# Jiang-Muyun/PointNet12

Measured on AMD Instinct MI355X. Metric: points/sec fwd+bwd, PointNet2 SemSeg B=16x4096 pts, higher is better.
Workload: dtype f32 (wide-layer products: exact bf16x3 operand splits, 6 bf16 MFMAs per fp32 product, fp32 accumulate)

## Files before the change

### pointnet12_amd/csrc/mlp_res.hip

```cpp
#include "mlp_loaders.h"
#include "split_bf16.h"
#include <algorithm>

int pn2_wide_fwd(const float *X, int ldx, const float *in_affine, const float *W, int ldw, const float *bias, float *Y, int ldy,
                 int64_t P, int K, int N, double *stats, LazyBn lz, hipStream_t s, int64_t *rows_done, int Kpool,
                 const float *pool_gamma, float *pool_ws);

namespace {

constexpr int RES_BM = 64;

struct ResPlan {
    signed char dx_rb[8], dx_cj[8];
    signed char dw_cj[8], dw_q0[8], dw_q1[8];
};

inline bool make_res_plan(int CI_T, ResPlan *out) {
    ResPlan p;
    int load[8], next_q[4] = {0, 0, 0, 0};
    for (int w = 0; w < 8; ++w) { p.dx_rb[w] = p.dx_cj[w] = -1; p.dw_cj[w] = 0; p.dw_q0[w] = p.dw_q1[w] = 0; load[w] = 0; }
    if (CI_T < 1 || CI_T > 4) return false;
    for (int i = 0; i < 2 * CI_T; ++i) { p.dx_rb[i] = (signed char)(i & 1); p.dx_cj[i] = (signed char)(i >> 1); load[i] = 2; }
    const int target = CI_T > 2 ? CI_T : 2;
    for (int pass = 0; pass < 2; ++pass)
// ... 686 lines not shown
                        const float4 a0 = xr[0], a1 = xr[1], a2 = xr[2];
                        g0[0] = __builtin_fmaf(dz, a0.x, g0[0]); g0[FUSE0 ? 1 : 0] = __builtin_fmaf(dz, a0.y, g0[FUSE0 ? 1 : 0]);
                        g0[FUSE0 ? 2 : 0] = __builtin_fmaf(dz, a0.z, g0[FUSE0 ? 2 : 0]); g0[FUSE0 ? 3 : 0] = __builtin_fmaf(dz, a0.w, g0[FUSE0 ? 3 : 0]);
                        g0[FUSE0 ? 4 : 0] = __builtin_fmaf(dz, a1.x, g0[FUSE0 ? 4 : 0]); g0[FUSE0 ? 5 : 0] = __builtin_fmaf(dz, a1.y, g0[FUSE0 ? 5 : 0]);
                        g0[FUSE0 ? 6 : 0] = __builtin_fmaf(dz, a1.z, g0[FUSE0 ? 6 : 0]); g0[FUSE0 ? 7 : 0] = __builtin_fmaf(dz, a1.w, g0[FUSE0 ? 7 : 0]);
                        g0[FUSE0 ? 8 : 0] = __builtin_fmaf(dz, a2.x, g0[FUSE0 ? 8 : 0]); g0[FUSE0 ? 9 : 0] = __builtin_fmaf(dz, a2.y, g0[FUSE0 ? 9 : 0]);
                        g0[FUSE0 ? 10 : 0] = __builtin_fmaf(dz, a2.z, g0[FUSE0 ? 10 : 0]); g0[FUSE0 ? 11 : 0] = __builtin_fmaf(dz, a2.w, g0[FUSE0 ? 11 : 0]);
                    } else {
#if defined(PN2_EXP_NOSTORE)
                        if (dz == 1.2345e-33f) xb[offx] = dz;
#elif defined(PN2_EXP_PLAINSTORE)
                        xb[offx] = dz;
#else
                        PN2_STREAM_STORE(dz, xb + offx);
#endif
                    }
                    offx += ((r & 3) == 3 ? 5u : 1u) * (unsigned)ldxo;
                }
                if (MASKED) { st0 += (double)s0; st1 += (double)s1; }
                RSTAMP(4)
            }
            chunk += G;
            buf ^= 1;
        };
        while (chunk < chunks) {
            iter(D2 ? raw1 : raw0);
            if (chunk >= chunks) break;
            iter(raw0);
        }
        RSTAMP_FLUSH(wave)
        RABS(wave, 2)
        if (!DXW) {
#pragma unroll
            for (int j = 0; j < TW; ++j) {
                const int e = (wave - CI_T) + j * NDW;
                if (e < NTILE) {
                    const int mb = e / CI_T, nb = e - mb * CI_T;
#pragma unroll
                    for (int r = 0; r < 16; ++r)
                        atomicAdd(dW + (int64_t)(mb * 32 + acc_row(r, lh)) * lddw + nb * 32 + l31, accw[DXW ? 0 : j][r]);
                }
            }
        } else if (MASKED && red_p != nullptr) {
            st0 += __shfl_xor(st0, 32, 64);
            st1 += __shfl_xor(st1, 32, 64);
            if (lh == 0) {
                double *rep = red_p + (size_t)(blockIdx.x % PN2_STAT_REPLICAS) * 2 * Ci;
                atomicAdd(rep + ecol, st0);
                atomicAdd(rep + Ci + ecol, st1);
            }
        }
        if (DXW && FUSE0) {
#pragma unroll
            for (int j = 0; j < (DXW && FUSE0 ? 12 : 1); ++j) g0[j] += __shfl_xor(g0[j], 32, 64);
            if (lh == 0) {
                float *pr = part0 + ((size_t)(blockIdx.x % PN2_CF_REPL) * Ci + ecol) * 16;
#pragma unroll
                for (int j = 0; j < (DXW && FUSE0 ? 12 : 1); ++j) atomicAdd(pr + j, g0[j]);
            }
        }
    };
    if (has_dx) run(pn2_true{}); else run(pn2_false{});
    RABS(wave, 3)
}

template <int CO_T, int CI_T, bool POOLED, bool MASKED, bool FUSE0 = false>
int launch_split_bwd_res(ResDy dy, const float *Yp, int ldp, const float *aff_p, const float *W, int ldw, int64_t tiles, float *dX, int ldxo,
                         double *red_p, float *dW, int lddw, hipStream_t s, const float *X0 = nullptr, int ld0 = 0, float *part0 = nullptr) {
    constexpr int Co = 32 * CO_T, Ci = 32 * CI_T;
    constexpr size_t lds = 2 * 6 * (size_t)(32 * 256) + sizeof(float) * (2 * 32 * (Ci + 4) + 8 * Co + 6 * Ci + (FUSE0 ? 2 * 32 * 12 : 0)) +
                           (CO_T == 4 && CI_T < 4 ? (size_t)CI_T * (Co / 16) * 1024 : 0);
    static_assert(lds <= 160 * 1024, "LDS");
    if ((reinterpret_cast<uintptr_t>(dy.Y) & 15) != 0 || (reinterpret_cast<uintptr_t>(Yp) & 15) != 0) return PN2_EUNSUPPORTED;
    auto kern = split_bwd_res_kernel<CO_T, CI_T, POOLED, MASKED, FUSE0>;
    static Pn2PerDevice raised;
    if (pn2_raise_dynamic_lds(reinterpret_cast<const void *>(kern), raised) != PN2_OK) return PN2_ELAUNCH;
    const int64_t chunks = tiles * (RES_BM / 32), cap = pn2_num_cus();
    PN2_NOTE_KERNEL(kern);
    hipLaunchKernelGGL(kern, dim3((unsigned)(chunks < cap ? chunks : cap)), dim3(512), lds, s, dy, Yp, ldp, aff_p, W, ldw, chunks, dX, ldxo,
                       red_p, dW, lddw, X0, ld0, part0);
    return pn2_launch_status();
}

template <int CO_T, int CI_T>
__global__ __launch_bounds__(512, 1) void split_bwd_cf_kernel(const float *dZp, const int32_t *arg, int ldo, int kshift, const float *W2 ,
                                                              const float *Yp, int ldp, const float *aff_p, int64_t chunks, float *dX, int ldxo, double *red_p,
                                                              float *slab) {
    constexpr int Co = 32 * CO_T, Ci = 32 * CI_T, BP = 32, QD = Co / 4, QP = Ci / 4, LDP = Ci + 4;
    constexpr int PANEL = BP * 256, BUF = 6 * PANEL;
    constexpr int KBX = Co / 16, KBM = Ci / 16, KBT = KBX + KBM;
    constexpr int NS = 8 - CI_T - 1, NTS = 64 * NS;
    constexpr int NGT = CI_T * (CI_T + 1) / 2, LDT = Co + Ci + 4;
    static_assert(NS >= CO_T, "one staging wave per D column");
    constexpr int RPP = NTS / QD, IT_D = (BP + RPP - 1) / RPP, IT_P = (BP * QP + NTS - 1) / NTS;
    static_assert(NTS % QD == 0, "one channel quad of D per staging thread");
    unsigned char *lds_b = reinterpret_cast<unsigned char *>(res_lds);
    float *Yps = res_lds + (2 * BUF) / 4;
    float *xtab = Yps + 2 * BP * LDP;
    const int t = threadIdx.x, lane = t & 63, wave = __builtin_amdgcn_readfirstlane(t >> 6), l31 = lane & 31, lh = lane >> 5;
    const int G = gridDim.x;
    RABS(wave, 0)
    for (int i = t; i < 3 * Ci; i += 512) { const float v = aff_p[i]; xtab[i] = v; xtab[3 * Ci + i] = i < Ci ? v : -v; }

    const bool has_dx = wave < CI_T, is_gram = wave == CI_T;
    const int ecol = (has_dx ? wave : 0) * 32 + l31;
    const int ts = wave <= CI_T ? 0 : t - 64 * (CI_T + 1);
    struct Raw { float4 z; int4 a; float4 p[IT_P]; };
    Raw raw;
    auto p_item = [&](int i, int &row, int &q) { const int idx = (NTS * (i + 1) > BP * QP) ? min(ts + NTS * i, BP * QP - 1) : ts + NTS * i; row = idx / QP; q = idx - row * QP; };
    auto fetch = [&](int64_t chunk) {
        const unsigned m0 = (unsigned)(chunk < chunks ? chunk : chunks - 1) * BP;
        const unsigned o = (m0 >> kshift) * (unsigned)ldo + 4u * (unsigned)(ts % QD);
        raw.z = ld4(dZp + o);
        raw.a = ld4i(arg + o);
#pragma unroll
        for (int i = 0; i < IT_P; ++i) {
            int row, q;
            p_item(i, row, q);
            raw.p[i] = ld4(Yp + ((m0 + (unsigned)row) * (unsigned)ldp + 4u * (unsigned)q));
        }
    };
    auto store_split = [&](unsigned char *img, int row, int q, const float4 v) {
        unsigned h0, m0, l0, h1, m1, l1;
        split2(v.x, v.y, h0, m0, l0);
        split2(v.z, v.w, h1, m1, l1);
        const unsigned o = tr_img_off(row, q >> 1) + 8u * (unsigned)(q & 1);
        *reinterpret_cast<uint2 *>(img + o) = make_uint2(h0, h1);
        *reinterpret_cast<uint2 *>(img + o + PANEL) = make_uint2(m0, m1);
        *reinterpret_cast<uint2 *>(img + o + 2 * PANEL) = make_uint2(l0, l1);
    };
    auto stage = [&](int64_t chunk, int buf) {
        unsigned char *ia = lds_b + buf * BUF, *ib = ia + 3 * PANEL;
        float *yp = Yps + buf * (BP * LDP);
        const unsigned m0 = (unsigned)(chunk < chunks ? chunk : chunks - 1) * BP;
        const int kbase = (int)(m0 & ((1u << kshift) - 1u));
        const int par = (int)(chunk & 1);
        const float *xt = xtab + par * (3 * Ci);
        const float lim = par ? -INFINITY : INFINITY;
        {
            unsigned h0, m0_, l0, h1, m1, l1;
            split2(raw.z.x, raw.z.y, h0, m0_, l0);
            split2(raw.z.z, raw.z.w, h1, m1, l1);
            const unsigned sm2 = par ? 0x80008000u : 0u;
            h0 ^= sm2; m0_ ^= sm2; l0 ^= sm2; h1 ^= sm2; m1 ^= sm2; l1 ^= sm2;
            const int q = ts % QD, r0 = ts / QD;
            const int4 a = raw.a;
#pragma unroll
            for (int i = 0; i < IT_D; ++i) {
                const int row = (RPP * (i + 1) > BP) ? min(r0 + RPP * i, BP - 1) : r0 + RPP * i;
                const int k = kbase + row;
                const unsigned k0 = (a.x == k ? 0x0000ffffu : 0u) | (a.y == k ? 0xffff0000u : 0u);
                const unsigned k1 = (a.z == k ? 0x0000ffffu : 0u) | (a.w == k ? 0xffff0000u : 0u);
                const unsigned o = tr_img_off(row, q >> 1) + 8u * (unsigned)(q & 1);
                *reinterpret_cast<uint2 *>(ia + o) = make_uint2(h0 & k0, h1 & k1);
                *reinterpret_cast<uint2 *>(ia + o + PANEL) = make_uint2(m0_ & k0, m1 & k1);
                *reinterpret_cast<uint2 *>(ia + o + 2 * PANEL) = make_uint2(l0 & k0, l1 & k1);
            }
        }
#pragma unroll
        for (int i = 0; i < IT_P; ++i) {
            int row, q;
            p_item(i, row, q);
            float4 x = raw.p[i];
            *reinterpret_cast<float4 *>(&yp[row * LDP + 4 * q]) = x;
            const float4 mu = *reinterpret_cast<const float4 *>(&xt[4 * q]), sc = *reinterpret_cast<const float4 *>(&xt[Ci + 4 * q]);
            const float4 be = *reinterpret_cast<const float4 *>(&xt[2 * Ci + 4 * q]);
            x.x = __builtin_amdgcn_fmed3f(bn_act(x.x, mu.x, sc.x, be.x), 0.f, lim); x.y = __builtin_amdgcn_fmed3f(bn_act(x.y, mu.y, sc.y, be.y), 0.f, lim);
            x.z = __builtin_amdgcn_fmed3f(bn_act(x.z, mu.z, sc.z, be.z), 0.f, lim); x.w = __builtin_amdgcn_fmed3f(bn_act(x.w, mu.w, sc.w, be.w), 0.f, lim);
            store_split(ib, row, q, x);
        }
    };
    auto raw_landed = [&]() {
        asm volatile("" : "+v"(raw.z.x), "+v"(raw.z.y), "+v"(raw.z.z), "+v"(raw.z.w));
        asm volatile("" : "+v"(raw.a.x), "+v"(raw.a.y), "+v"(raw.a.z), "+v"(raw.a.w));
#pragma unroll
        for (int i = 0; i < IT_P; ++i) asm volatile("" : "+v"(raw.p[i].x), "+v"(raw.p[i].y), "+v"(raw.p[i].z), "+v"(raw.p[i].w));
    };
    const int g16 = lane >> 4, j16 = lane & 15, tq = j16 >> 2, tp = j16 & 3;
    auto frag_t = [&](const unsigned char *img, int cblk, int pb) {
        const int c0 = (cblk * 32 + 16 * (g16 & 1)) >> 3;
        SplitFrag f;
#pragma unroll
        for (int r2 = 0; r2 < 2; ++r2) {
            const int row = 16 * pb + 8 * (g16 >> 1) + 4 * r2 + tq;
            const unsigned o = tr_img_off(row, c0 + (tp >> 1)) + 8u * (unsigned)(tp & 1);
            const pn2_s16x4 v = __builtin_amdgcn_ds_read_tr16_b64_v4i16(
                reinterpret_cast<__attribute__((address_space(3))) pn2_s16x4 *>((__attribute__((address_space(3))) unsigned char *)(img) + o));
            const uint2 u = __builtin_bit_cast(uint2, v);
            f.u[2 * r2] = u.x; f.u[2 * r2 + 1] = u.y;
        }
        return f;
    };

    if (has_dx) {
        SplitFrag wh[KBT], wm[KBT], wl[KBM];
        uint4 *wl_lds = reinterpret_cast<uint4 *>(xtab + 6 * Ci) + (size_t)wave * KBX * 64 + lane;
        {
            float v[KBT][8];
#pragma unroll
            for (int kb = 0; kb < KBT; ++kb)
#pragma unroll
                for (int e = 0; e < 8; ++e) v[kb][e] = W2[(16 * kb + 8 * lh + e) * Ci + ecol];
#pragma unroll
            for (int kb = 0; kb < KBT; ++kb) {
                SplitFrag lo;
#pragma unroll
                for (int e = 0; e < 4; ++e) split2(v[kb][2 * e], v[kb][2 * e + 1], wh[kb].u[e], wm[kb].u[e], lo.u[e]);
                if (kb < KBX) wl_lds[kb * 64] = lo.q; else wl[kb < KBX ? 0 : kb - KBX] = lo;
            }
        }
        Affine a(aff_p, Ci);
        const float emu = a.mean[ecol], esc = a.scale[ecol], ebe = a.beta[ecol], eis = a.invstd[ecol];
        const float eh = W2[(Co + Ci) * Ci + ecol];
        double st0 = 0.0, st1 = 0.0, st2 = 0.0;
        int64_t chunk = blockIdx.x;
        int buf = 0;
        __syncthreads();
        RABS(wave, 1)
        RSTAMP_DECL
        while (chunk < chunks) {
            __syncthreads();
            RSTAMP(2)
            const unsigned char *ia = lds_b + buf * BUF, *ib = ia + 3 * PANEL;
            f32x16 acc, acc2;
#pragma unroll
            for (int r = 0; r < 16; ++r) { acc[r] = 0.f; acc2[r] = 0.f; }
#ifndef PN2_X_CF_NODXM
#pragma unroll
            for (int kb = 0; kb < KBT; ++kb) {
                const unsigned char *img = kb < KBX ? ia : ib;
                const unsigned o = tr_img_off(l31, 2 * (kb < KBX ? kb : kb - KBX) + lh);
                SplitFrag ah, am, al, wlo;
                ah.q = *reinterpret_cast<const uint4 *>(img + o);
                am.q = *reinterpret_cast<const uint4 *>(img + o + PANEL);
                al.q = *reinterpret_cast<const uint4 *>(img + o + 2 * PANEL);
                if (kb < KBX) wlo.q = wl_lds[kb * 64]; else wlo = wl[kb < KBX ? 0 : kb - KBX];
                acc = __builtin_amdgcn_mfma_f32_32x32x16_bf16(al.v, wh[kb].v, acc, 0, 0, 0);
                acc2 = __builtin_amdgcn_mfma_f32_32x32x16_bf16(ah.v, wlo.v, acc2, 0, 0, 0);
                acc = __builtin_amdgcn_mfma_f32_32x32x16_bf16(am.v, wm[kb].v, acc, 0, 0, 0);
                acc2 = __builtin_amdgcn_mfma_f32_32x32x16_bf16(am.v, wh[kb].v, acc2, 0, 0, 0);
                acc = __builtin_amdgcn_mfma_f32_32x32x16_bf16(ah.v, wm[kb].v, acc, 0, 0, 0);
                acc2 = __builtin_amdgcn_mfma_f32_32x32x16_bf16(ah.v, wh[kb].v, acc2, 0, 0, 0);
            }
#endif
#ifdef PN2_STAMP
            { float a0_ = acc[0] + acc2[0]; asm volatile("" : "+v"(a0_)); }
#endif
            RSTAMP(3)
#ifdef PN2_X_CF_NOEPI
            if (acc[0] == 1.2345e-33f) dX[0] = acc2[1];
            chunk += G; buf ^= 1;
            continue;
#endif
            const float *yq = Yps + buf * (BP * LDP) + (4 * lh) * LDP + ecol;
            float yv[16];
#pragma unroll
            for (int r = 0; r < 16; ++r) yv[r] = yq[((r & 3) + 8 * (r >> 2)) * LDP];
            float *xb = dX + ((size_t)chunk * BP + 4 * lh) * (unsigned)ldxo;
            unsigned offx = (unsigned)ecol;
            asm volatile("" : "+v"(offx));
            float s0 = 0.f, s1 = 0.f, s2 = 0.f;
            const unsigned sgn = (unsigned)(chunk & 1) << 31;
#pragma unroll
            for (int r = 0; r < 16; ++r) {
                const float y = yv[r];
                const float x = bn_act(y, emu, esc, ebe);
                float dz = __uint_as_float(__float_as_uint(acc[r] + acc2[r]) ^ sgn) + eh;
                dz = x > 0.f ? dz : 0.f;
                s0 += dz;
                s1 = __builtin_fmaf(dz, (y - emu) * eis, s1);
                s2 += fmaxf(x, 0.f);
                PN2_STREAM_STORE(dz, xb + offx);
                offx += ((r & 3) == 3 ? 5u : 1u) * (unsigned)ldxo;
            }
            st0 += (double)s0; st1 += (double)s1; st2 += (double)s2;
            RSTAMP(4)
            chunk += G;
            buf ^= 1;
        }
        RSTAMP_FLUSH(wave)
        RABS(wave, 2)
        st0 += __shfl_xor(st0, 32, 64);
        st1 += __shfl_xor(st1, 32, 64);
        st2 += __shfl_xor(st2, 32, 64);
        if (lh == 0) {
            if (red_p != nullptr) {
                double *rep = red_p + (size_t)(blockIdx.x % PN2_STAT_REPLICAS) * 2 * Ci;
                atomicAdd(rep + ecol, st0);
                atomicAdd(rep + Ci + ecol, st1);
            }
            slab[(size_t)blockIdx.x * (Ci * LDT) + (size_t)ecol * LDT + Co + Ci] = (float)st2;
        }
    } else {
        constexpr int PA[6] = {2, 0, 1, 1, 0, 0}, PB[6] = {0, 2, 1, 0, 1, 0};
        auto mm2 = [&](f32x16 &c0, const SplitFrag (&a0)[3], const SplitFrag (&b0)[3], f32x16 &c1, const SplitFrag (&a1)[3], const SplitFrag (&b1)[3]) {
#pragma unroll
            for (int q = 0; q < 6; ++q) {
                c0 = __builtin_amdgcn_mfma_f32_32x32x16_bf16(a0[PA[q]].v, b0[PB[q]].v, c0, 0, 0, 0);
                c1 = __builtin_amdgcn_mfma_f32_32x32x16_bf16(a1[PA[q]].v, b1[PB[q]].v, c1, 0, 0, 0);
            }
        };
        auto mm1 = [&](f32x16 &c0, const SplitFrag (&a0)[3], const SplitFrag (&b0)[3]) {
#pragma unroll
            for (int q = 0; q < 6; ++q) c0 = __builtin_amdgcn_mfma_f32_32x32x16_bf16(a0[PA[q]].v, b0[PB[q]].v, c0, 0, 0, 0);
        };
        auto frag3 = [&](const unsigned char *img, int blk, int pb, SplitFrag (&f)[3]) {
            f[0] = frag_t(img, blk, pb); f[1] = frag_t(img + PANEL, blk, pb); f[2] = frag_t(img + 2 * PANEL, blk, pb);
        };
        float *sl = slab + (size_t)blockIdx.x * (Ci * LDT);
        if (is_gram) {
            f32x16 accg[NGT];
#pragma unroll
            for (int j = 0; j < NGT; ++j)
#pragma unroll
                for (int r = 0; r < 16; ++r) accg[j][r] = 0.f;
            int64_t chunk = blockIdx.x;
            int buf = 0;
            __syncthreads();
            RABS(wave, 1)
            RSTAMP_DECL
            while (chunk < chunks) {
                __syncthreads();
                RSTAMP(2)
#ifndef PN2_X_CF_NOT
                const unsigned char *ib = lds_b + buf * BUF + 3 * PANEL;
#pragma unroll
                for (int pb = 0; pb < BP / 16; ++pb) {
                    SplitFrag fx[CI_T][3];
#pragma unroll
                    for (int i = 0; i < CI_T; ++i) frag3(ib, i, pb, fx[i]);
                    if constexpr (CI_T == 1) {
                        mm1(accg[0], fx[0], fx[0]);
                    } else if constexpr (CI_T == 2) {
                        mm2(accg[0], fx[0], fx[0], accg[1], fx[0], fx[1]);
                        mm1(accg[2], fx[1], fx[1]);
                    } else {
                        static_assert(CI_T <= 3, "Gram tiles");
                        mm2(accg[0], fx[0], fx[0], accg[1], fx[0], fx[1]);
                        mm2(accg[2], fx[1], fx[1], accg[3], fx[0], fx[2]);
                        mm2(accg[4], fx[1], fx[2], accg[5], fx[2], fx[2]);
                    }
                }
#endif
                RSTAMP(3)
                chunk += G;
                buf ^= 1;
            }
            RSTAMP_FLUSH(wave)
            RABS(wave, 2)
#pragma unroll
            for (int j = 0; j < CI_T; ++j)
#pragma unroll
                for (int i = 0; i <= j; ++i) {
                    const f32x16 &acc = accg[j * (j + 1) / 2 + i];
#pragma unroll
                    for (int r = 0; r < 16; ++r) sl[(i * 32 + acc_row(r, lh)) * LDT + Co + j * 32 + l31] = acc[r];
                    if (i != j) {
#pragma unroll
                        for (int r = 0; r < 16; ++r) sl[(j * 32 + l31) * LDT + Co + i * 32 + acc_row(r, lh)] = acc[r];
                    }
                }
        } else {
            f32x16 accw[CI_T];
#pragma unroll
            for (int j = 0; j < CI_T; ++j)
#pragma unroll
                for (int r = 0; r < 16; ++r) accw[j][r] = 0.f;
            const int nb = wave - CI_T - 1 < CO_T ? wave - CI_T - 1 : -1;
            int64_t chunk = blockIdx.x;
            fetch(chunk);
            __syncthreads();
            stage(chunk, 0);
            fetch(chunk + G);
            raw_landed();
            int buf = 0;
            RABS(wave, 1)
            RSTAMP_DECL
            while (chunk < chunks) {
                __syncthreads();
                RSTAMP(2)
#ifndef PN2_X_CF_NOSTAGE
                stage(chunk + G, buf ^ 1);
#endif
                RSTAMP(0)
#ifndef PN2_X_CF_NOFETCH
                fetch(chunk + 2 * (int64_t)G);
#endif
                __builtin_amdgcn_sched_barrier(0);
                RSTAMP(1)
#ifndef PN2_X_CF_NOT
                if (nb >= 0) {
                    const unsigned char *ia = lds_b + buf * BUF, *ib = ia + 3 * PANEL;
#pragma unroll
                    for (int pb = 0; pb < BP / 16; ++pb) {
                        SplitFrag fb[3], fa0[3], fa1[3];
                        frag3(ia, nb, pb, fb);
                        frag3(ib, 0, pb, fa0);
                        if constexpr (CI_T >= 2) {
                            frag3(ib, 1, pb, fa1);
                            mm2(accw[0], fa0, fb, accw[CI_T >= 2 ? 1 : 0], fa1, fb);
                            if constexpr (CI_T == 3) {
                                frag3(ib, 2, pb, fa0);
                                mm1(accw[CI_T == 3 ? 2 : 0], fa0, fb);
                            }
                        } else {
                            mm1(accw[0], fa0, fb);
                        }
                    }
                }
#endif
                RSTAMP(3)
                chunk += G;
                buf ^= 1;
            }
            RSTAMP_FLUSH(wave)
            RABS(wave, 2)
            if (nb >= 0) {
#pragma unroll
                for (int i = 0; i < CI_T; ++i)
#pragma unroll
                    for (int r = 0; r < 16; ++r) sl[(i * 32 + acc_row(r, lh)) * LDT + nb * 32 + l31] = accw[i][r];
            }
        }
    }
    RABS(wave, 3)
}

__global__ __launch_bounds__(128) void cf_prep_kernel(LazyCoef lc, const float *coef, int ldc, const float *__restrict__ W, int ldw,
                                                      const float *__restrict__ bias, int Co, int Ci, float *__restrict__ W2) {
    __shared__ double fac[256];
    lazy_coef_prologue(lc);
    const float *c0 = coef, *q1 = coef + ldc, *q0 = coef + 2 * ldc, *mean = coef + 3 * ldc;
    const int r = blockIdx.x;
    if (r < Co) {
        for (int i = threadIdx.x; i < Ci; i += 128) W2[r * Ci + i] = c0[r] * W[(int64_t)r * ldw + i];
        return;
    }
    const int j = r - Co;
    for (int c = threadIdx.x; c < Co; c += 128)
        fac[c] = j == Ci ? ((double)q1[c] * ((double)bias[c] - (double)mean[c]) + (double)q0[c]) : (double)W[(int64_t)c * ldw + j] * (double)q1[c];
    __syncthreads();
    for (int i = threadIdx.x; i < Ci; i += 128) {
        double s0 = 0.0, s1 = 0.0, s2 = 0.0, s3 = 0.0;
#pragma unroll 4
        for (int c = 0; c < Co; c += 4) {
            s0 += fac[c] * (double)W[(int64_t)c * ldw + i];
            s1 += fac[c + 1] * (double)W[(int64_t)(c + 1) * ldw + i];
            s2 += fac[c + 2] * (double)W[(int64_t)(c + 2) * ldw + i];
            s3 += fac[c + 3] * (double)W[(int64_t)(c + 3) * ldw + i];
        }
        W2[r * Ci + i] = (float)((s0 + s1) + (s2 + s3));
    }
}

__global__ __launch_bounds__(256) void cf_finish_kernel(const float *__restrict__ slab, int nslab, int Co, int Ci, const float *coef, int ldc,
                                                        const float *__restrict__ W, int ldw, const float *__restrict__ bias,
                                                        float *__restrict__ dW, int lddw) {
    extern __shared__ double cf_row[];
    const int i = blockIdx.x, LDT = Co + Ci + 4, NQ = LDT / 4;
    const int q = threadIdx.x & 63, sg = threadIdx.x >> 6;
    double a0 = 0.0, a1 = 0.0, a2 = 0.0, a3 = 0.0;
    if (q < NQ) {
        const float *p = slab + (size_t)i * LDT + 4 * q;
        const size_t ss = (size_t)Ci * LDT;
        int w = sg;
        for (; w + 28 < nslab; w += 32) {
            float4 v[8];
#pragma unroll
            for (int e = 0; e < 8; ++e) v[e] = ld4(p + (size_t)(w + 4 * e) * ss);
#pragma unroll
            for (int e = 0; e < 8; ++e) { a0 += (double)v[e].x; a1 += (double)v[e].y; a2 += (double)v[e].z; a3 += (double)v[e].w; }
        }
        for (; w < nslab; w += 4) {
            const float4 v = ld4(p + (size_t)w * ss);
            a0 += (double)v.x; a1 += (double)v.y; a2 += (double)v.z; a3 += (double)v.w;
        }
        double *d = cf_row + sg * LDT + 4 * q;
        d[0] = a0; d[1] = a1; d[2] = a2; d[3] = a3;
    }
    __syncthreads();
    for (int n = threadIdx.x; n < LDT; n += 256) cf_row[n] = (cf_row[n] + cf_row[LDT + n]) + (cf_row[2 * LDT + n] + cf_row[3 * LDT + n]);
    __syncthreads();
    const float *c0 = coef, *q1 = coef + ldc, *q0 = coef + 2 * ldc, *mean = coef + 3 * ldc;
    const double sx = cf_row[Co + Ci];
    for (int c = threadIdx.x; c < Co; c += 256) {
        double dot = 0.0;
        for (int j = 0; j < Ci; ++j) dot += (double)W[(int64_t)c * ldw + j] * cf_row[Co + j];
        const double g = (double)c0[c] * cf_row[c] + (double)q1[c] * (dot + ((double)bias[c] - (double)mean[c]) * sx) + (double)q0[c] * sx;
        dW[(int64_t)c * lddw + i] += (float)g;
    }
}

template <int CO_T, int CI_T>
int launch_split_bwd_cf(const float *dZp, const int32_t *arg, int ldo, int kshift, const float *coef, LazyCoef lc, const float *W, int ldw,
                        const float *bias, const float *Yp, int ldp, const float *aff_p, int64_t P, float *dX, int ldxo, double *red_p,
                        float *dW, int lddw, float *scratch, hipStream_t s) {
    constexpr int Co = 32 * CO_T, Ci = 32 * CI_T, LDT = Co + Ci + 4;
    constexpr size_t lds = 2 * 6 * (size_t)(32 * 256) + sizeof(float) * (2 * 32 * (Ci + 4) + 6 * Ci) + (size_t)CI_T * (Co / 16) * 1024;
    static_assert(lds <= 160 * 1024, "LDS");
    auto kern = split_bwd_cf_kernel<CO_T, CI_T>;
    static Pn2PerDevice raised;
    if (pn2_raise_dynamic_lds(reinterpret_cast<const void *>(kern), raised) != PN2_OK) return PN2_ELAUNCH;
    float *W2 = scratch, *slab = scratch + (((Co + Ci + 1) * Ci + 63) & ~63);
    const int64_t chunks = P / 32, cap = pn2_num_cus() < 256 ? pn2_num_cus() : 256;
    const int grid = (int)(chunks < cap ? chunks : cap);
    hipLaunchKernelGGL(cf_prep_kernel, dim3(Co + Ci + 1), dim3(128), 0, s, lc, coef, (Co + 3) & ~3, W, ldw, bias, Co, Ci, W2);
    PN2_NOTE_KERNEL(kern);
    hipLaunchKernelGGL(kern, dim3((unsigned)grid), dim3(512), lds, s, dZp, arg, ldo, kshift, W2, Yp, ldp, aff_p, chunks, dX, ldxo, red_p, slab);
    hipLaunchKernelGGL(cf_finish_kernel, dim3(Ci), dim3(256), sizeof(double) * 4 * LDT, s, slab, grid, Co, Ci, coef, (Co + 3) & ~3, W, ldw, bias,
                       dW, lddw);
    return pn2_launch_status();
}

#define PN2_RES_CASE(CO, CI, POOL, MASKED)                                                                                \
    if (Co == CO && Ci == CI)                                                                                              \
        return launch_bwd_res<CO / 32, CI / 32, POOL, MASKED>(dy, Yp, ldp, aff_p, W, ldw, tiles, dX, ldxo, red_p, dW, lddw, s);

int dispatch_bwd_res(int Kpool, bool masked, int Co, int Ci, ResDy dy, const float *Yp, int ldp, const float *aff_p, const float *W,
                     int ldw, int64_t tiles, float *dX, int ldxo, double *red_p, float *dW, int lddw, hipStream_t s) {
    if (pn2_opt(PN2_OPT_SPLIT) && pn2_opt(PN2_OPT_SPLIT_RES)) {
#define PN2_SPLIT_RES_CASE(CO, CI, POOLED, MASKED)                                                                        \
        if (Co == CO && Ci == CI) {                                                                                        \
            const int rc = launch_split_bwd_res<CO / 32, CI / 32, POOLED, MASKED>(dy, Yp, ldp, aff_p, W, ldw, tiles, dX, ldxo, red_p, dW, lddw, s); \
            if (rc != PN2_EUNSUPPORTED) return rc;                                                                         \
        }
        const bool all = pn2_opt(PN2_OPT_SPLIT_RES) >= 2;
        if (Kpool == 0 && masked) {
            if (all) { PN2_SPLIT_RES_CASE(32, 32, false, true) }
            PN2_SPLIT_RES_CASE(64, 64, false, true) PN2_SPLIT_RES_CASE(96, 64, false, true)
            if (tiles >= pn2_opt(PN2_OPT_SPLIT_RES_MIN_TILES_128)) { PN2_SPLIT_RES_CASE(128, 128, false, true) }
        } else if (Kpool == 0) {
            if (tiles >= pn2_opt(PN2_OPT_SPLIT_RES_MIN_TILES_128)) { PN2_SPLIT_RES_CASE(128, 128, false, false) }
        } else if (masked && Kpool % 32 == 0) {
            if (all) { PN2_SPLIT_RES_CASE(64, 32, true, true) }
            PN2_SPLIT_RES_CASE(128, 64, true, true) PN2_SPLIT_RES_CASE(128, 96, true, true)
        }
#undef PN2_SPLIT_RES_CASE
    }
    if (Kpool == 0 && masked) {
        PN2_RES_CASE(32, 32, 0, true) PN2_RES_CASE(64, 64, 0, true) PN2_RES_CASE(96, 64, 0, true)
        if (tiles >= 4096) { PN2_RES_CASE(128, 128, 0, true) }
    } else if (Kpool == 0) {
        if (tiles >= 4096) { PN2_RES_CASE(128, 128, 0, false) }
    } else if (masked && Kpool % 64 == 0) {
        PN2_RES_CASE(128, 64, 1, true) PN2_RES_CASE(128, 96, 1, true)
    } else if (masked && Kpool == 32) {
        PN2_RES_CASE(64, 32, 2, true) PN2_RES_CASE(128, 64, 2, true)
    }
    return PN2_EUNSUPPORTED;
}

struct ResPool {
    float2 *rec;
    const float *gamma;
    int ldp, U;
    LazyBn lz;
};

template <int K_T, int N_T, bool ACT, int POOL>
__global__ __launch_bounds__(512, 2) void fwd_res_kernel(const float *__restrict__ X, int ldx, const float *aff ,
                                                         const float *__restrict__ W, int ldw, const float *__restrict__ bias,
                                                         float *__restrict__ Y, int ldy, int64_t slabs, double *__restrict__ stats,
                                                         ResPool pool) {
    constexpr int K = 32 * K_T, N = 32 * N_T, LDA = K + 4, QK = K / 4, IT = 32 * QK / 64;
    const int NW = blockDim.x >> 6;
    float *Ws = res_lds;
    float *atab = Ws + N * LDA;
    const int t = threadIdx.x, lane = t & 63, wave = __builtin_amdgcn_readfirstlane(t >> 6), l31 = lane & 31, lh = lane >> 5;
    float *Ab = atab + 3 * K + wave * (32 * LDA);
    RABS(wave, 0)

    lazy_bn_prologue(pool.lz);
    for (int i = t; i < N * QK; i += blockDim.x) {
        const int n = i / QK, q = i - n * QK;
        const float *src = W + (int64_t)n * ldw + 4 * q;
        float4 v;
        if ((ldw & 3) == 0 && (reinterpret_cast<uintptr_t>(W) & 15) == 0) v = ld4(src);
        else v = make_float4(src[0], src[1], src[2], src[3]);
        *reinterpret_cast<float4 *>(&Ws[n * LDA + 4 * q]) = v;
    }
    if (ACT)
        for (int i = t; i < 3 * K; i += blockDim.x) atab[i] = aff[i];
    float bj[N_T];
// ... 326 lines not shown

extern "C" int pn2_bn_pool_select(const float *pool_ws, const float *affine, int64_t G, int C, float *out, int ldo, int32_t *arg,
                                  const pn2_bn_lazy *lazy, pn2_stream_t stream) {
    PN2_CHECK_ARG(lazy_bn_ok(lazy, affine, C));
    PN2_CHECK_ARG(pool_ws && affine && out && arg && G > 0 && C > 0 && C % 32 == 0 && ldo >= C && ldo % 4 == 0 &&
                  (reinterpret_cast<uintptr_t>(pool_ws) & 15) == 0 && (reinterpret_cast<uintptr_t>(out) & 15) == 0);
    const int64_t n = G * (C >> 2);
    int64_t blocks = pn2_cdiv(n, 256);
    const int64_t cap = (int64_t)pn2_num_cus() * 8;
    if (blocks > cap) blocks = cap;
    hipLaunchKernelGGL(bn_pool_select_kernel, dim3((unsigned)blocks), dim3(256), 0, pn2_s(stream),
                       reinterpret_cast<const float2 *>(pool_ws), C, affine, C, G, C, out, ldo, arg, make_lazy_bn(lazy));
    return pn2_launch_status();
}

extern "C" int pn2_conv1x1_bwd(const float *dZ, int ldz, const float *dZp, int ldo, const int32_t *arg, int Kpool, const float *Y,
                               int ldy, const float *coef, const float *W, int ldw, const float *prev_Y, int ld_prev,
                               const float *prev_affine, float *dXout, int ldxo, double *prev_red, float *dW, int lddw,
                               int64_t P, int C_out, int C_in, const pn2_bn_coef_lazy *coef_lazy, pn2_stream_t stream) {
    PN2_CHECK_ARG(Y && coef && W && prev_Y && dXout && dW && P > 0 && P < (1LL << 31) && res_shape_ok(C_out, C_in));
    PN2_CHECK_ARG(lazy_coef_ok(coef_lazy, coef, C_out));
    PN2_CHECK_ARG(dZ != nullptr || (dZp && arg && Kpool > 0));
    PN2_CHECK_ARG(ldw >= C_in && lddw >= C_in && ldy % 4 == 0 && ldy >= C_out && ld_prev % 4 == 0 && ld_prev >= C_in && ldxo >= C_in);
    PN2_CHECK_ARG(prev_affine != nullptr || prev_red == nullptr);
    hipStream_t s = pn2_s(stream);
    const int kshift = dZ ? 0 : pow2_shift(Kpool);
    PN2_CHECK_ARG(dZ ? (ldz == ldy) : (kshift >= 0 && ldo % 4 == 0 && ldo >= C_out && prev_affine != nullptr && P % Kpool == 0));
    int64_t tiles = P / RES_BM, P_full = tiles * RES_BM;
    int rc = PN2_OK;
    const int64_t ld_max = std::max(std::max((int64_t)ldy, (int64_t)ld_prev), std::max((int64_t)ldxo, dZ ? (int64_t)ldz : (int64_t)ldo));
    if (P * ld_max >= (1LL << 32)) { tiles = 0; P_full = 0; }
    if (tiles > 0) {
        ResDy dy{dZ, dZp, arg, ldo, kshift, Y, ldy, coef, make_lazy_coef(coef_lazy)};
        rc = dispatch_bwd_res(dZ ? 0 : Kpool, prev_affine != nullptr, C_out, C_in, dy, prev_Y, ld_prev, prev_affine, W, ldw, tiles, dXout, ldxo,
                              prev_red, dW, lddw, s);
        if (rc == PN2_EUNSUPPORTED) { rc = PN2_OK; tiles = 0; P_full = 0; }
        else coef_lazy = nullptr;
    }
    if (rc != PN2_OK || P_full == P) return rc;
    const int64_t tail = P - P_full;
    const int64_t g_off = dZ ? 0 : (P_full / Kpool) * ldo;
    const float *dZt = dZ ? dZ + P_full * ldz : nullptr;
    const float *dZpt = dZ ? nullptr : dZp + g_off;
    const int32_t *argt = dZ ? nullptr : arg + g_off;
    rc = pn2_conv1x1_dgrad(dZt, ldz, dZpt, ldo, argt, Kpool, Y + P_full * ldy, ldy, coef, W, ldw, prev_affine ? prev_Y + P_full * ld_prev : nullptr,
                           ld_prev, prev_affine, dXout + P_full * ldxo, ldxo, prev_red, tail, C_out, C_in, nullptr, coef_lazy, stream);
    if (rc != PN2_OK) return rc;
    return pn2_conv1x1_wgrad(dZt, ldz, dZpt, ldo, argt, Kpool, Y + P_full * ldy, ldy, coef, prev_Y + P_full * ld_prev, ld_prev, prev_affine,
                             dW, lddw, nullptr, tail, C_out, C_in, nullptr, stream);
}

static bool cf_shape(int C_out, int C_in) { return C_out == 128 && (C_in == 96 || C_in == 64); }

extern "C" int pn2_conv1x1_bwd_cf_supported(int64_t P, int C_out, int C_in, int Kpool) {
    if (!(pn2_opt(PN2_OPT_SPLIT) && pn2_opt(PN2_OPT_SPLIT_RES) && pn2_opt(PN2_OPT_POOL_CF))) return 0;
    if (!pn2_res_supported(P, C_out, C_in) || !cf_shape(C_out, C_in)) return 0;
    if (C_in == 64 && pn2_opt(PN2_OPT_POOL_CF) < 2) return 0;
    if (Kpool < 32 || (Kpool & (Kpool - 1)) != 0 || P % Kpool != 0) return 0;
    if (P * (int64_t)std::max(C_out, C_in) >= (1LL << 32)) return 0;
    return 1;
}

extern "C" int64_t pn2_conv1x1_bwd_cf_scratch_bytes(int C_out, int C_in) {
    if (!cf_shape(C_out, C_in)) return 0;
    const int64_t w2 = (((int64_t)(C_out + C_in + 1) * C_in + 63) & ~63LL);
    return 4 * (w2 + 256LL * C_in * (C_out + C_in + 4));
}

extern "C" int pn2_conv1x1_bwd_cf(const float *dZp, int ldo, const int32_t *arg, int Kpool, const float *coef, const float *W, int ldw,
                                  const float *bias, const float *prev_Y, int ld_prev, const float *prev_affine, float *dXout, int ldxo,
                                  double *prev_red, float *dW, int lddw, int64_t P, int C_out, int C_in, const pn2_bn_coef_lazy *coef_lazy,
                                  float *scratch, pn2_stream_t stream) {
    PN2_CHECK_ARG(dZp && arg && coef && W && bias && prev_Y && prev_affine && dXout && dW && scratch && P > 0 && P < (1LL << 31));
    PN2_CHECK_ARG(lazy_coef_ok(coef_lazy, coef, C_out));
    PN2_CHECK_ARG(ldw >= C_in && lddw >= C_in && ld_prev % 4 == 0 && ld_prev >= C_in && ldxo >= C_in && ldo % 4 == 0 && ldo >= C_out);
    PN2_CHECK_ARG((reinterpret_cast<uintptr_t>(scratch) & 255) == 0 && (reinterpret_cast<uintptr_t>(prev_Y) & 15) == 0 &&
                  (reinterpret_cast<uintptr_t>(dZp) & 15) == 0 && (reinterpret_cast<uintptr_t>(arg) & 15) == 0);
    if (!pn2_conv1x1_bwd_cf_supported(P, C_out, C_in, Kpool)) return PN2_EUNSUPPORTED;
    const int64_t ld_max = std::max(std::max((int64_t)ld_prev, (int64_t)ldxo), (int64_t)ldo);
    if (P * ld_max >= (1LL << 32)) return PN2_EUNSUPPORTED;
    const int kshift = pow2_shift(Kpool);
    const LazyCoef lc = make_lazy_coef(coef_lazy);
    hipStream_t s = pn2_s(stream);
    if (C_in == 96) return launch_split_bwd_cf<4, 3>(dZp, arg, ldo, kshift, coef, lc, W, ldw, bias, prev_Y, ld_prev, prev_affine, P, dXout, ldxo, prev_red, dW, lddw, scratch, s);
    return launch_split_bwd_cf<4, 2>(dZp, arg, ldo, kshift, coef, lc, W, ldw, bias, prev_Y, ld_prev, prev_affine, P, dXout, ldxo, prev_red, dW, lddw, scratch, s);
}

extern "C" int pn2_conv1x1_bwd_first_supported(int64_t P, int C_out, int C_in, int N0) {
    if (!(pn2_opt(PN2_OPT_SPLIT) && pn2_opt(PN2_OPT_SPLIT_RES) && pn2_opt(PN2_OPT_FUSE_FIRST))) return 0;
    if (!pn2_res_supported(P, C_out, C_in) || P % 64 != 0 || N0 < 1 || N0 > 12) return 0;
    if (P * (int64_t)std::max(C_out, C_in) >= (1LL << 32)) return 0;
    return (C_out == 96 && C_in == 64) || (C_out == 64 && C_in == 64);
}

extern "C" int pn2_conv1x1_bwd_first(const float *dZ, int ldz, const float *Y, int ldy, const float *coef, const float *W, int ldw,
                                     const float *prev_Y, int ld_prev, const float *prev_affine, double *prev_red, float *dW, int lddw,
                                     const float *X0, int ld0, int N0, void *cf_scratch, int64_t P, int C_out, int C_in,
                                     const pn2_bn_coef_lazy *coef_lazy, pn2_stream_t stream) {
    PN2_CHECK_ARG(dZ && Y && coef && W && prev_Y && prev_affine && prev_red && dW && X0 && cf_scratch && P > 0 && P < (1LL << 31));
    PN2_CHECK_ARG(lazy_coef_ok(coef_lazy, coef, C_out));
    PN2_CHECK_ARG(ldz == ldy && ldw >= C_in && lddw >= C_in && ldy % 4 == 0 && ldy >= C_out && ld_prev % 4 == 0 && ld_prev >= C_in);
    PN2_CHECK_ARG(ld0 % 4 == 0 && ld0 >= 12 && (reinterpret_cast<uintptr_t>(X0) & 15) == 0 && (reinterpret_cast<uintptr_t>(cf_scratch) & 15) == 0);
    if (!pn2_conv1x1_bwd_first_supported(P, C_out, C_in, N0)) return PN2_EUNSUPPORTED;
    if (P * (int64_t)std::max((int64_t)ldy, std::max((int64_t)ld_prev, (int64_t)ld0)) >= (1LL << 32)) return PN2_EUNSUPPORTED;
    float *part0 = reinterpret_cast<float *>(reinterpret_cast<double *>(cf_scratch) + PN2_CF_REPL * 256);
    ResDy dy{dZ, nullptr, nullptr, 0, 0, Y, ldy, coef, make_lazy_coef(coef_lazy)};
    const int64_t tiles = P / RES_BM;
    hipStream_t s = pn2_s(stream);
    if (C_out == 96) return launch_split_bwd_res<3, 2, false, true, true>(dy, prev_Y, ld_prev, prev_affine, W, ldw, tiles, nullptr, 0, prev_red, dW, lddw, s, X0, ld0, part0);
    return launch_split_bwd_res<2, 2, false, true, true>(dy, prev_Y, ld_prev, prev_affine, W, ldw, tiles, nullptr, 0, prev_red, dW, lddw, s, X0, ld0, part0);
}
```

### pointnet12_amd/csrc/pn2_common.h

```cpp
#pragma once
#include <hip/hip_runtime.h>
#include <stdint.h>
#include <mutex>
#include <set>
#include <utility>
#include "../../include/pn2.h"

#define PN2_WAVE 64
#define PN2_CF_REPL 8

#ifdef PN2_PLAIN_STORES
#define PN2_STREAM_STORE(value, ptr) (*(ptr) = (value))
#else
#define PN2_STREAM_STORE(value, ptr) __builtin_nontemporal_store((value), (ptr))
#endif

#define PN2_CHECK_ARG(cond) \
    do {                    \
        if (!(cond)) return PN2_EINVAL; \
    } while (0)

static inline int pn2_launch_status() { return hipGetLastError() == hipSuccess ? PN2_OK : PN2_ELAUNCH; }

static inline hipStream_t pn2_s(pn2_stream_t s) { return reinterpret_cast<hipStream_t>(s); }

static inline int64_t pn2_cdiv(int64_t a, int64_t b) { return (a + b - 1) / b; }

#define PN2_OPTION_LIST(X) \
    X(FPS_ROWS_MIN_PPT, 24)  \
    X(FPS_ROWMAP, 2)  \
    X(FPS_SINGLE_MAX, 24576)  \
    X(FPS_PIECE, 0)  \
    X(FPS_COOP, 1)  \
    X(FPS_PRUNE, 1)  \
    X(BQ_ORDER, 1)  \
    X(FEWROW_MAX_TILES, 1024)  \
    X(FEWROW_MAX_TILES_DGRAD, 512)  \
    X(FEWROW_KS, 0)  \
    X(NT_CFG, 0)  \
    X(NT_SMALL_DEPTH, 1)  \
    X(NT_NSPLIT, 1)  \
    X(TN_SPLITDIV, 1)  \
    X(TN_CFG, 0)  \
    X(TN_NARROW, 1)  \
    X(TN_SMALLP, 65536)  \
    X(TN_SMALL_DEPTH, 2)  \
    X(CF_WGS_PER_CU, 2)  \
    X(WGRAD_SKINNY, 1)  \
    X(BWD_PAIR, 1)  \
    X(RES, 1)  \
    X(RES_MIN_ROWS, 32768)  \
    X(RES_HALF, 1)  \
    X(WIDE, 1)  \
    X(WIDE_MIN_ROWS, 65536)  \
    X(SPLIT, 1)  \
    X(SPLIT_WGRAD, 1)  \
    X(SPLIT_K256, 1)  \
    X(SPLIT_NARROW, 1)  \
    X(SPLIT_RES, 1)  \
    X(FUSE_FIRST, 1)  \
    X(SPLIT_WG2, 1)  \
    X(POOL_CF, 2)  \
    X(SPLIT_RES_MIN_TILES_128, 1024)  \
    X(SPLIT_MIN_ROWS_128, 98304)  \
    X(RING, 0)  \
    X(WIDE_POOL, 1)  \
    X(WIDE_ADB196, 1)  \
    X(WIDE_WGRAD, 1)  \
    X(WIDE_WGRAD_MIN_ROWS, 131072)  \
    X(WGRAD_TWO_PHASE, 0)  \
    X(WGRAD_TWO_PHASE_ALL, 0)  \
    X(SEG_CHUNK, 0)

enum Pn2Option {
#define PN2_X(name, dflt) PN2_OPT_##name,
    PN2_OPTION_LIST(PN2_X)
#undef PN2_X
    PN2_OPT_COUNT
};
extern int pn2_option_table[PN2_OPT_COUNT];
static inline int pn2_opt(int id) { return __atomic_load_n(&pn2_option_table[id], __ATOMIC_RELAXED); }

extern thread_local const void *pn2_last_kernel_fn;
#define PN2_NOTE_KERNEL(...) (pn2_last_kernel_fn = reinterpret_cast<const void *>(__VA_ARGS__))

#define PN2_MAX_DEVICES 16
static inline int pn2_device_slot() {
    int dev = 0;
    if (hipGetDevice(&dev) != hipSuccess || dev < 0) dev = 0;
    return dev < PN2_MAX_DEVICES ? dev : PN2_MAX_DEVICES - 1;
}

static inline int pn2_num_cus() {
    static int cus[PN2_MAX_DEVICES] = {0};
    const int slot = pn2_device_slot();
    if (cus[slot] == 0) {
        int dev = 0;
        hipDeviceProp_t prop;
        int n = 0;
        if (hipGetDevice(&dev) == hipSuccess && hipGetDeviceProperties(&prop, dev) == hipSuccess) n = prop.multiProcessorCount;
        cus[slot] = n > 0 ? n : 256;
    }
    return cus[slot];
}

struct Pn2PerDevice {
    bool flag[PN2_MAX_DEVICES] = {false};
    bool get() const { return flag[pn2_device_slot()]; }
    void set() { flag[pn2_device_slot()] = true; }
};
static inline int pn2_raise_dynamic_lds(const void *kernel, Pn2PerDevice &done) {
    if (done.get()) return PN2_OK;
    if (hipFuncSetAttribute(kernel, hipFuncAttributeMaxDynamicSharedMemorySize, 160 * 1024) != hipSuccess) return PN2_ELAUNCH;
    done.set();
    return PN2_OK;
}

static inline int pn2_raise_dynamic_lds_once(const void *kernel) {
    static std::mutex mu;
    static std::set<std::pair<const void *, int>> done;
    const std::pair<const void *, int> key(kernel, pn2_device_slot());
    std::lock_guard<std::mutex> lock(mu);
    if (done.count(key)) return PN2_OK;
    if (hipFuncSetAttribute(kernel, hipFuncAttributeMaxDynamicSharedMemorySize, 160 * 1024) != hipSuccess) return PN2_ELAUNCH;
    done.insert(key);
    return PN2_OK;
}

#define PN2_OPAQUE1(a) asm volatile("" : "+v"(a))
#define PN2_OPAQUE3(a, b, c) asm volatile("" : "+v"(a), "+v"(b), "+v"(c))
#define PN2_OPAQUE4(a, b, c, d) asm volatile("" : "+v"(a), "+v"(b), "+v"(c), "+v"(d))

__device__ __forceinline__ unsigned long long pn2_wave_max_u64(unsigned long long v) {
#pragma unroll
    for (int m = 32; m >= 1; m >>= 1) {
        unsigned long long o = __shfl_xor(v, m, 64);
        v = o > v ? o : v;
    }
    return v;
}

__device__ __forceinline__ unsigned pn2_row_max_u32(unsigned v) {
    asm volatile("s_nop 1\n\t"
                 "v_max_u32_dpp %0, %0, %0 quad_perm:[1,0,3,2] row_mask:0xf bank_mask:0xf\n\t"
                 "s_nop 1\n\t"
// ... 71 lines not shown
```

Measured before the change: 13.11 million.

## Add sparse max-pool backward path to fused conv backward kernel

Adds a SPARSE variant of the fused pooled-conv backward kernel, enabled by default. It exploits the fact that the max-pool gradient is nonzero in only one row per channel. Instead of staging a dense masked dZ image and running split-bf16 MFMAs over it, the kernel scatters dZ·W2 contributions with scalar FMAs from an LDS copy of W2. The weight-gradient contribution is likewise accumulated only for the argmax rows. This cuts MFMA work and LDS image size. The cost is serialized ballot loops, possible divergence, and extra LDS for W2 and the S buffer.

```diff
diff --git a/pointnet12_amd/csrc/mlp_res.hip b/pointnet12_amd/csrc/mlp_res.hip
--- a/pointnet12_amd/csrc/mlp_res.hip
+++ b/pointnet12_amd/csrc/mlp_res.hip
@@ -792,25 +792,32 @@
     return pn2_launch_status();
 }
 
-template <int CO_T, int CI_T>
+template <int CO_T, int CI_T, bool SPARSE>
 __global__ __launch_bounds__(512, 1) void split_bwd_cf_kernel(const float *dZp, const int32_t *arg, int ldo, int kshift, const float *W2 ,
                                                               const float *Yp, int ldp, const float *aff_p, int64_t chunks, float *dX, int ldxo, double *red_p,
                                                               float *slab) {
     constexpr int Co = 32 * CO_T, Ci = 32 * CI_T, BP = 32, QD = Co / 4, QP = Ci / 4, LDP = Ci + 4;
-    constexpr int PANEL = BP * 256, BUF = 6 * PANEL;
+    constexpr int PANEL = BP * 256, BUF = (SPARSE ? 3 : 6) * PANEL;
     constexpr int KBX = Co / 16, KBM = Ci / 16, KBT = KBX + KBM;
+    constexpr int KB0 = SPARSE ? KBX : 0;
     constexpr int NS = 8 - CI_T - 1, NTS = 64 * NS;
     constexpr int NGT = CI_T * (CI_T + 1) / 2, LDT = Co + Ci + 4;
+    constexpr int CPL = (Ci + 63) / 64, CIS = Ci / 4;
     static_assert(NS >= CO_T, "one staging wave per D column");
+    static_assert(!SPARSE || (Co == 128 && CO_T == 4 && CIS % 4 == 0), "SPARSE: two channels per lane, four S / T waves");
     constexpr int RPP = NTS / QD, IT_D = (BP + RPP - 1) / RPP, IT_P = (BP * QP + NTS - 1) / NTS;
     static_assert(NTS % QD == 0, "one channel quad of D per staging thread");
     unsigned char *lds_b = reinterpret_cast<unsigned char *>(res_lds);
     float *Yps = res_lds + (2 * BUF) / 4;
     float *xtab = Yps + 2 * BP * LDP;
+    float *W2s = xtab + 6 * Ci, *Ss = W2s + Co * Ci;
+    auto ximg = [&](int b) { return lds_b + b * BUF + (SPARSE ? 0 : 3 * PANEL); };
     const int t = threadIdx.x, lane = t & 63, wave = __builtin_amdgcn_readfirstlane(t >> 6), l31 = lane & 31, lh = lane >> 5;
     const int G = gridDim.x;
     RABS(wave, 0)
     for (int i = t; i < 3 * Ci; i += 512) { const float v = aff_p[i]; xtab[i] = v; xtab[3 * Ci + i] = i < Ci ? v : -v; }
+    if constexpr (SPARSE)
+        for (int i = t; i < Co * Ci / 4; i += 512) reinterpret_cast<float4 *>(W2s)[i] = ld4(W2 + 4 * i);
 
     const bool has_dx = wave < CI_T, is_gram = wave == CI_T;
     const int ecol = (has_dx ? wave : 0) * 32 + l31;
@@ -820,9 +827,15 @@
     auto p_item = [&](int i, int &row, int &q) { const int idx = (NTS * (i + 1) > BP * QP) ? min(ts + NTS * i, BP * QP - 1) : ts + NTS * i; row = idx / QP; q = idx - row * QP; };
     auto fetch = [&](int64_t chunk) {
         const unsigned m0 = (unsigned)(chunk < chunks ? chunk : chunks - 1) * BP;
-        const unsigned o = (m0 >> kshift) * (unsigned)ldo + 4u * (unsigned)(ts % QD);
-        raw.z = ld4(dZp + o);
-        raw.a = ld4i(arg + o);
+        if constexpr (SPARSE) {
+            const unsigned o = (m0 >> kshift) * (unsigned)ldo + (unsigned)lane;
+            raw.z = make_float4(dZp[o], dZp[o + 64], 0.f, 0.f);
+            raw.a = make_int4(arg[o], arg[o + 64], 0, 0);
+        } else {
+            const unsigned o = (m0 >> kshift) * (unsigned)ldo + 4u * (unsigned)(ts % QD);
+            raw.z = ld4(dZp + o);
+            raw.a = ld4i(arg + o);
+        }
 #pragma unroll
         for (int i = 0; i < IT_P; ++i) {
             int row, q;
@@ -839,15 +852,55 @@
         *reinterpret_cast<uint2 *>(img + o + PANEL) = make_uint2(m0, m1);
         *reinterpret_cast<uint2 *>(img + o + 2 * PANEL) = make_uint2(l0, l1);
     };
+    auto d_rows = [&](int64_t chunk) {
+        const unsigned kbase = ((unsigned)(chunk < chunks ? chunk : chunks - 1) * BP) & ((1u << kshift) - 1u);
+        return make_uint2((unsigned)raw.a.x - kbase, (unsigned)raw.a.y - kbase);
+    };
     auto stage = [&](int64_t chunk, int buf) {
-        unsigned char *ia = lds_b + buf * BUF, *ib = ia + 3 * PANEL;
+        unsigned char *ia = lds_b + buf * BUF, *ib = ximg(buf);
         float *yp = Yps + buf * (BP * LDP);
         const unsigned m0 = (unsigned)(chunk < chunks ? chunk : chunks - 1) * BP;
         const int kbase = (int)(m0 & ((1u << kshift) - 1u));
         const int par = (int)(chunk & 1);
         const float *xt = xtab + par * (3 * Ci);
         const float lim = par ? -INFINITY : INFINITY;
-        {
+        if constexpr (SPARSE) {
+            const int sw = wave - CI_T - 1;
+            if (sw < 4) {
+                const uint2 rw = d_rows(chunk);
+                float sacc[8][CPL];
+#pragma unroll
+                for (int rr = 0; rr < 8; ++rr)
+#pragma unroll
+                    for (int j = 0; j < CPL; ++j) sacc[rr][j] = 0.f;
+                int col[CPL];
+#pragma unroll
+                for (int j = 0; j < CPL; ++j) col[j] = min(lane + 64 * j, Ci - 1);
+#pragma unroll
+                for (int rr = 0; rr < 8; ++rr) {
+                    const unsigned r = (unsigned)(8 * sw + rr);
+#pragma unroll
+                    for (int h = 0; h < 2; ++h) {
+                        unsigned long long m = __ballot((h ? rw.y : rw.x) == r);
+                        const int dzb = __float_as_int(h ? raw.z.y : raw.z.x);
+                        while (m) {
+                            const int l = __builtin_ctzll(m);
+                            m &= m - 1;
+                            const float d = __int_as_float(__builtin_amdgcn_readlane(dzb, l));
+                            const float *w = W2s + (64 * h + l) * Ci;
+#pragma unroll
+                            for (int j = 0; j < CPL; ++j) sacc[rr][j] = __builtin_fmaf(d, w[col[j]], sacc[rr][j]);
+                        }
+                    }
+                }
+                float *sp = Ss + buf * (BP * Ci) + (8 * sw) * Ci;
+#pragma unroll
+                for (int rr = 0; rr < 8; ++rr)
+#pragma unroll
+                    for (int j = 0; j < CPL; ++j)
+                        if (lane + 64 * j < Ci) sp[rr * Ci + lane + 64 * j] = sacc[rr][j];
+            }
+        } else {
             unsigned h0, m0_, l0, h1, m1, l1;
             split2(raw.z.x, raw.z.y, h0, m0_, l0);
             split2(raw.z.z, raw.z.w, h1, m1, l1);
@@ -908,11 +961,11 @@
         {
             float v[KBT][8];
 #pragma unroll
-            for (int kb = 0; kb < KBT; ++kb)
+            for (int kb = KB0; kb < KBT; ++kb)
 #pragma unroll
                 for (int e = 0; e < 8; ++e) v[kb][e] = W2[(16 * kb + 8 * lh + e) * Ci + ecol];
 #pragma unroll
-            for (int kb = 0; kb < KBT; ++kb) {
+            for (int kb = KB0; kb < KBT; ++kb) {
                 SplitFrag lo;
 #pragma unroll
                 for (int e = 0; e < 4; ++e) split2(v[kb][2 * e], v[kb][2 * e + 1], wh[kb].u[e], wm[kb].u[e], lo.u[e]);
@@ -931,13 +984,13 @@
         while (chunk < chunks) {
             __syncthreads();
             RSTAMP(2)
-            const unsigned char *ia = lds_b + buf * BUF, *ib = ia + 3 * PANEL;
+            const unsigned char *ia = lds_b + buf * BUF, *ib = ximg(buf);
             f32x16 acc, acc2;
 #pragma unroll
             for (int r = 0; r < 16; ++r) { acc[r] = 0.f; acc2[r] = 0.f; }
 #ifndef PN2_X_CF_NODXM
 #pragma unroll
-            for (int kb = 0; kb < KBT; ++kb) {
+            for (int kb = KB0; kb < KBT; ++kb) {
                 const unsigned char *img = kb < KBX ? ia : ib;
                 const unsigned o = tr_img_off(l31, 2 * (kb < KBX ? kb : kb - KBX) + lh);
                 SplitFrag ah, am, al, wlo;
@@ -966,6 +1019,9 @@
             float yv[16];
 #pragma unroll
             for (int r = 0; r < 16; ++r) yv[r] = yq[((r & 3) + 8 * (r >> 2)) * LDP];
+            float sv[16];
+#pragma unroll
+            for (int r = 0; r < 16; ++r) sv[r] = SPARSE ? Ss[buf * (BP * Ci) + ((r & 3) + 8 * (r >> 2) + 4 * lh) * Ci + ecol] : 0.f;
             float *xb = dX + ((size_t)chunk * BP + 4 * lh) * (unsigned)ldxo;
             unsigned offx = (unsigned)ecol;
             asm volatile("" : "+v"(offx));
@@ -975,7 +1031,9 @@
             for (int r = 0; r < 16; ++r) {
                 const float y = yv[r];
                 const float x = bn_act(y, emu, esc, ebe);
-                float dz = __uint_as_float(__float_as_uint(acc[r] + acc2[r]) ^ sgn) + eh;
+                float dz = __uint_as_float(__float_as_uint(acc[r] + acc2[r]) ^ sgn);
+                if constexpr (SPARSE) dz += sv[r];
+                dz += eh;
                 dz = x > 0.f ? dz : 0.f;
                 s0 += dz;
                 s1 = __builtin_fmaf(dz, (y - emu) * eis, s1);
@@ -1033,7 +1091,7 @@
                 __syncthreads();
                 RSTAMP(2)
 #ifndef PN2_X_CF_NOT
-                const unsigned char *ib = lds_b + buf * BUF + 3 * PANEL;
+                const unsigned char *ib = ximg(buf);
 #pragma unroll
                 for (int pb = 0; pb < BP / 16; ++pb) {
                     SplitFrag fx[CI_T][3];
@@ -1077,10 +1135,18 @@
 #pragma unroll
                 for (int r = 0; r < 16; ++r) accw[j][r] = 0.f;
             const int nb = wave - CI_T - 1 < CO_T ? wave - CI_T - 1 : -1;
+            float tacc[2][CIS];
+#pragma unroll
+            for (int h = 0; h < 2; ++h)
+#pragma unroll
+                for (int j = 0; j < CIS; ++j) tacc[h][j] = 0.f;
+            uint2 drow;
+            float2 dzv;
             int64_t chunk = blockIdx.x;
             fetch(chunk);
             __syncthreads();
             stage(chunk, 0);
+            if constexpr (SPARSE) { drow = d_rows(chunk); dzv = make_float2(raw.z.x, raw.z.y); }
             fetch(chunk + G);
             raw_landed();
             int buf = 0;
@@ -1092,6 +1158,9 @@
 #ifndef PN2_X_CF_NOSTAGE
                 stage(chunk + G, buf ^ 1);
 #endif
+                uint2 drow_n;
+                float2 dzv_n;
+                if constexpr (SPARSE) { drow_n = d_rows(chunk + G); dzv_n = make_float2(raw.z.x, raw.z.y); }
                 RSTAMP(0)
 #ifndef PN2_X_CF_NOFETCH
                 fetch(chunk + 2 * (int64_t)G);
@@ -1099,7 +1168,31 @@
                 __builtin_amdgcn_sched_barrier(0);
                 RSTAMP(1)
 #ifndef PN2_X_CF_NOT
-                if (nb >= 0) {
+                if constexpr (SPARSE) {
+                    if (nb >= 0) {
+                        const float *yb = Yps + buf * (BP * LDP) + nb * CIS;
+                        const float *mt = xtab + nb * CIS;
+#pragma unroll
+                        for (int h = 0; h < 2; ++h) {
+                            const unsigned r = h ? drow.y : drow.x;
+                            const bool hit = r < (unsigned)BP;
+                            if (__ballot(hit) != 0ull) {
+                                const float d = hit ? (h ? dzv.y : dzv.x) : 0.f;
+                                const float *yr = yb + (hit ? r : 0u) * LDP;
+#pragma unroll
+                                for (int q = 0; q < CIS / 4; ++q) {
+                                    const float4 y = ld4(yr + 4 * q), mu = ld4(mt + 4 * q), sc = ld4(mt + Ci + 4 * q), be = ld4(mt + 2 * Ci + 4 * q);
+                                    tacc[h][4 * q + 0] = __builtin_fmaf(d, fmaxf(bn_act(y.x, mu.x, sc.x, be.x), 0.f), tacc[h][4 * q + 0]);
+                                    tacc[h][4 * q + 1] = __builtin_fmaf(d, fmaxf(bn_act(y.y, mu.y, sc.y, be.y), 0.f), tacc[h][4 * q + 1]);
+                                    tacc[h][4 * q + 2] = __builtin_fmaf(d, fmaxf(bn_act(y.z, mu.z, sc.z, be.z), 0.f), tacc[h][4 * q + 2]);
+                                    tacc[h][4 * q + 3] = __builtin_fmaf(d, fmaxf(bn_act(y.w, mu.w, sc.w, be.w), 0.f), tacc[h][4 * q + 3]);
+                                }
+                            }
+                        }
+                    }
+                    drow = drow_n;
+                    dzv = dzv_n;
+                } else if (nb >= 0) {
                     const unsigned char *ia = lds_b + buf * BUF, *ib = ia + 3 * PANEL;
 #pragma unroll
                     for (int pb = 0; pb < BP / 16; ++pb) {
@@ -1125,7 +1218,12 @@
             }
             RSTAMP_FLUSH(wave)
             RABS(wave, 2)
-            if (nb >= 0) {
+            if (SPARSE && nb >= 0) {
+#pragma unroll
+                for (int h = 0; h < 2; ++h)
+#pragma unroll
+                    for (int j = 0; j < CIS; ++j) sl[(nb * CIS + j) * LDT + 64 * h + lane] = tacc[h][j];
+            } else if (nb >= 0) {
 #pragma unroll
                 for (int i = 0; i < CI_T; ++i)
 #pragma unroll
@@ -1201,14 +1299,15 @@
     }
 }
 
-template <int CO_T, int CI_T>
+template <int CO_T, int CI_T, bool SPARSE>
 int launch_split_bwd_cf(const float *dZp, const int32_t *arg, int ldo, int kshift, const float *coef, LazyCoef lc, const float *W, int ldw,
                         const float *bias, const float *Yp, int ldp, const float *aff_p, int64_t P, float *dX, int ldxo, double *red_p,
                         float *dW, int lddw, float *scratch, hipStream_t s) {
     constexpr int Co = 32 * CO_T, Ci = 32 * CI_T, LDT = Co + Ci + 4;
-    constexpr size_t lds = 2 * 6 * (size_t)(32 * 256) + sizeof(float) * (2 * 32 * (Ci + 4) + 6 * Ci) + (size_t)CI_T * (Co / 16) * 1024;
+    constexpr size_t lds = SPARSE ? 2 * 3 * (size_t)(32 * 256) + sizeof(float) * (2 * 32 * (Ci + 4) + 6 * Ci + Co * Ci + 2 * 32 * Ci)
+                                  : 2 * 6 * (size_t)(32 * 256) + sizeof(float) * (2 * 32 * (Ci + 4) + 6 * Ci) + (size_t)CI_T * (Co / 16) * 1024;
     static_assert(lds <= 160 * 1024, "LDS");
-    auto kern = split_bwd_cf_kernel<CO_T, CI_T>;
+    auto kern = split_bwd_cf_kernel<CO_T, CI_T, SPARSE>;
     static Pn2PerDevice raised;
     if (pn2_raise_dynamic_lds(reinterpret_cast<const void *>(kern), raised) != PN2_OK) return PN2_ELAUNCH;
     float *W2 = scratch, *slab = scratch + (((Co + Ci + 1) * Ci + 63) & ~63);
@@ -1701,8 +1800,12 @@
     const int kshift = pow2_shift(Kpool);
     const LazyCoef lc = make_lazy_coef(coef_lazy);
     hipStream_t s = pn2_s(stream);
-    if (C_in == 96) return launch_split_bwd_cf<4, 3>(dZp, arg, ldo, kshift, coef, lc, W, ldw, bias, prev_Y, ld_prev, prev_affine, P, dXout, ldxo, prev_red, dW, lddw, scratch, s);
-    return launch_split_bwd_cf<4, 2>(dZp, arg, ldo, kshift, coef, lc, W, ldw, bias, prev_Y, ld_prev, prev_affine, P, dXout, ldxo, prev_red, dW, lddw, scratch, s);
+    const bool sparse = pn2_opt(PN2_OPT_CF_SPARSE) != 0;
+    if (C_in == 96)
+        return (sparse ? launch_split_bwd_cf<4, 3, true> : launch_split_bwd_cf<4, 3, false>)(dZp, arg, ldo, kshift, coef, lc, W, ldw, bias, prev_Y, ld_prev,
+                                                                                              prev_affine, P, dXout, ldxo, prev_red, dW, lddw, scratch, s);
+    return (sparse ? launch_split_bwd_cf<4, 2, true> : launch_split_bwd_cf<4, 2, false>)(dZp, arg, ldo, kshift, coef, lc, W, ldw, bias, prev_Y, ld_prev,
+                                                                                          prev_affine, P, dXout, ldxo, prev_red, dW, lddw, scratch, s);
 }
 
 extern "C" int pn2_conv1x1_bwd_first_supported(int64_t P, int C_out, int C_in, int N0) {
diff --git a/pointnet12_amd/csrc/pn2_common.h b/pointnet12_amd/csrc/pn2_common.h
--- a/pointnet12_amd/csrc/pn2_common.h
+++ b/pointnet12_amd/csrc/pn2_common.h
@@ -61,6 +61,7 @@
     X(FUSE_FIRST, 1)  \
     X(SPLIT_WG2, 1)  \
     X(POOL_CF, 2)  \
+    X(CF_SPARSE, 1)  \
     X(SPLIT_RES_MIN_TILES_128, 1024)  \
     X(SPLIT_MIN_ROWS_128, 98304)  \
     X(RING, 0)  \
```

Result: no change. 13.02 million, median of 6 (-0.7%).
